# schmidtjonathan/Climate2Weather

Measured on AMD Instinct MI355X. Metric: UNet denoise steps/sec (train fwd+bwd+allreduce+AdamW+EMA windows/s), higher is better.
Workload: dtype bf16; 1 GPU; configs/sda_unet.yml default net, 5 vars x window 13 = 65 ch, 128x128, bf16 training step, 128 windows/GPU/step; global_batch=128, parallelism=dp1, params=72132929

## Files before the change

### climate2weather_amd/csrc/attention_mfma.hip

```cpp
#include <cstdlib>
#include "knobs.h"
#include "launch.h"

namespace {

constexpr int T64 = 64;
constexpr int PP = 144;

typedef __attribute__((ext_vector_type(4))) short s16x4_t;
typedef __attribute__((address_space(3))) s16x4_t lds_s16x4_t;

__device__ __forceinline__ bf16x8_t tr_frag(const char* base, int pitch, int k0, int col0, int li, int lg) {
    const int q = li >> 2, pp = li & 3;
    const char* p0 = base + (k0 + 8 * lg + q) * pitch + (col0 + pp * 4) * 2;
    const s16x4_t lo = __builtin_amdgcn_ds_read_tr16_b64_v4i16((lds_s16x4_t*)p0);
    const s16x4_t hi = __builtin_amdgcn_ds_read_tr16_b64_v4i16((lds_s16x4_t*)(p0 + 4 * pitch));
    return (bf16x8_t){lo[0], lo[1], lo[2], lo[3], hi[0], hi[1], hi[2], hi[3]};
}

template <int CTRL>
__device__ __forceinline__ float dpp_get(float v) {
    return __int_as_float(__builtin_amdgcn_update_dpp(0, __float_as_int(v), CTRL, 0xf, 0xf, false));
}
__device__ __forceinline__ float row16_sum(float v) {
    v += dpp_get<0x128>(v);
    v += dpp_get<0x124>(v);
    v += dpp_get<0x122>(v);
    return v + dpp_get<0x121>(v);
}
__device__ __forceinline__ float row16_max(float v) {
    v = fmaxf(v, dpp_get<0x128>(v));
    v = fmaxf(v, dpp_get<0x124>(v));
    v = fmaxf(v, dpp_get<0x122>(v));
    return fmaxf(v, dpp_get<0x121>(v));
}

__device__ __forceinline__ void stage_rows(char* dst, int pitch, const bf16_t* src, int ld, int C) {
    const int nch = C >> 3;
    for (int i = threadIdx.x; i < T64 * nch; i += blockDim.x) {
        const int r = i / nch, c = i - r * nch;
        *(u32x4_t*)(dst + r * pitch + c * 16) = *(const u32x4_t*)(src + (size_t)r * ld + c * 8);
    }
}

template <typename T>
__device__ __forceinline__ void strip_abt(f32x4_t (&acc)[4], const bf16_t* a, int lda, const bf16_t* b, int ldb, int ks0, int ks1, int w, int li,
                                          int lg) {
    const bf16_t* ar = a + (size_t)(16 * w + li) * lda + 8 * lg;
    const bf16_t* br = b + (size_t)li * ldb + 8 * lg;
#pragma unroll 4
    for (int ks = ks0; ks < ks1; ++ks) {
        const bf16x8_t av = *(const bf16x8_t*)(ar + 32 * ks);
#pragma unroll
        for (int n = 0; n < 4; ++n) {
            const bf16x8_t bv = *(const bf16x8_t*)(br + (size_t)(16 * n) * ldb + 32 * ks);
            acc[n] = mfma16s<T>(av, bv, acc[n]);
        }
    }
}

__device__ __forceinline__ void strip_to_lds(char* X, int w, const f32x4_t (&acc)[4], int li, int lg) {
#pragma unroll
    for (int n = 0; n < 4; ++n)
#pragma unroll
        for (int r = 0; r < 4; ++r) *(float*)(X + w * 4096 + ((4 * lg + r) * 64 + 16 * n + li) * 4) = acc[n][r];
}
__device__ __forceinline__ void strip_from_lds(const char* X, int w, f32x4_t (&acc)[4], int li, int lg) {
#pragma unroll
    for (int n = 0; n < 4; ++n)
#pragma unroll
        for (int r = 0; r < 4; ++r) acc[n][r] = *(const float*)(X + w * 4096 + ((4 * lg + r) * 64 + 16 * n + li) * 4);
}

template <typename T>
__device__ __forceinline__ void strip_times_lds(bf16_t* out, int ldo, const bf16x8_t (&a)[2], const char* M, int pitch, int ct0, int ct1, int w,
                                                int li, int lg) {
    for (int ct = ct0; ct < ct1; ++ct) {
        f32x4_t acc = {0.f, 0.f, 0.f, 0.f};
#pragma unroll
        for (int ks = 0; ks < 2; ++ks) acc = mfma16s<T>(a[ks], tr_frag(M, pitch, 32 * ks, 16 * ct, li, lg), acc);
#pragma unroll
        for (int r = 0; r < 4; ++r) out[(size_t)(16 * w + 4 * lg + r) * ldo + 16 * ct + li] = f32_to_bits16<T>(acc[r]);
    }
}

constexpr int NTA = 512;

template <typename T>
__global__ __launch_bounds__(NTA) void attn_mfma_fwd_kernel(const bf16_t* __restrict__ qkv, bf16_t* __restrict__ o, float* __restrict__ lse,
                                                            int C, float scale2) {
    extern __shared__ __attribute__((aligned(16))) char smem[];
    const int VP = C * 2 + 16;
    char* const Vl = smem;
    char* const Pl = smem + T64 * VP;
    char* const X = Pl + T64 * PP;
    const int tid = threadIdx.x, lane = tid & 63, w8 = tid >> 6, w = w8 & 3, half = w8 >> 2, li = lane & 15, lg = lane >> 4;
    const int ld = 3 * C;
    const bf16_t* base = qkv + (size_t)blockIdx.x * T64 * ld;
    stage_rows(Vl, VP, base + 2 * C, ld, C);

    f32x4_t s[4] = {};
    const int nks = C / 32, ksm = nks / 2;
    strip_abt<T>(s, base, ld, base + C, ld, half ? ksm : 0, half ? nks : ksm, w, li, lg);
    if (half) strip_to_lds(X, w, s, li, lg);
    __syncthreads();
    if (!half) {
        f32x4_t s1[4];
        strip_from_lds(X, w, s1, li, lg);
#pragma unroll
        for (int r = 0; r < 4; ++r) {
            float m = -INFINITY;
#pragma unroll
            for (int n = 0; n < 4; ++n) {
                s[n][r] = (s[n][r] + s1[n][r]) * scale2;
                m = fmaxf(m, s[n][r]);
            }
            m = row16_max(m);
            float sum = 0.f;
#pragma unroll
            for (int n = 0; n < 4; ++n) {
                s[n][r] = __expf(s[n][r] - m);
                sum += s[n][r];
            }
            sum = row16_sum(sum);
            const float inv = 1.0f / sum;
            const int row = 16 * w + 4 * lg + r;
#pragma unroll
            for (int n = 0; n < 4; ++n) *(bf16_t*)(Pl + row * PP + (16 * n + li) * 2) = f32_to_bits16<T>(s[n][r] * inv);
            if (lse != nullptr && li == 0) lse[(size_t)blockIdx.x * T64 + row] = m + __logf(sum);
        }
    }
    __syncthreads();
    bf16x8_t pa[2];
#pragma unroll
    for (int ks = 0; ks < 2; ++ks) pa[ks] = *(const bf16x8_t*)(Pl + (16 * w + li) * PP + (32 * ks + 8 * lg) * 2);
    const int nct = C / 16, ctm = nct / 2;
    strip_times_lds<T>(o + (size_t)blockIdx.x * T64 * C, C, pa, Vl, VP, half ? ctm : 0, half ? nct : ctm, w, li, lg);
}

template <typename T>
__global__ __launch_bounds__(NTA) void attn_mfma_bwd_kernel(const bf16_t* __restrict__ qkv, const bf16_t* __restrict__ d_o,
                                                            const float* __restrict__ lse, bf16_t* __restrict__ dqkv, int C, float scale2) {
    extern __shared__ __attribute__((aligned(16))) char smem[];
    const int VP = C * 2 + 16;
    char* const B0 = smem;
    char* const B1 = smem + T64 * VP;
    char* const Pl = smem + 2 * T64 * VP;
    char* const Sl = Pl + T64 * PP;
    char* const X = Pl;
    const int tid = threadIdx.x, lane = tid & 63, w8 = tid >> 6, w = w8 & 3, half = w8 >> 2, li = lane & 15, lg = lane >> 4;
    const int ld = 3 * C;
    const bf16_t* base = qkv + (size_t)blockIdx.x * T64 * ld;
    const bf16_t* dob = d_o + (size_t)blockIdx.x * T64 * C;
    bf16_t* dbase = dqkv + (size_t)blockIdx.x * T64 * ld;
    stage_rows(B0, VP, base + C, ld, C);
    stage_rows(B1, VP, dob, C, C);

    f32x4_t s[4] = {}, dp[4];
    if (!half) strip_abt<T>(s, base, ld, base + C, ld, 0, C / 32, w, li, lg);
    else strip_abt<T>(s, dob, C, base + 2 * C, ld, 0, C / 32, w, li, lg);
    if (half) strip_to_lds(X, w, s, li, lg);
    __syncthreads();
    if (!half) strip_from_lds(X, w, dp, li, lg);
    __syncthreads();
    if (!half) {
#pragma unroll
        for (int r = 0; r < 4; ++r) {
            const int row = 16 * w + 4 * lg + r;
            const float l = lse[(size_t)blockIdx.x * T64 + row];
            float delta = 0.f;
#pragma unroll
            for (int n = 0; n < 4; ++n) {
                s[n][r] = __expf(s[n][r] * scale2 - l);
                delta += s[n][r] * dp[n][r];
            }
            delta = row16_sum(delta);
#pragma unroll
            for (int n = 0; n < 4; ++n) {
                const float ds = s[n][r] * (dp[n][r] - delta) * scale2;
                *(bf16_t*)(Pl + row * PP + (16 * n + li) * 2) = f32_to_bits16<T>(s[n][r]);
                *(bf16_t*)(Sl + row * PP + (16 * n + li) * 2) = f32_to_bits16<T>(ds);
            }
        }
    }
    __syncthreads();
    const int nct = C / 16, ctm = nct / 2, ct0 = half ? ctm : 0, ct1 = half ? nct : ctm;
    bf16x8_t a[2];
#pragma unroll
    for (int ks = 0; ks < 2; ++ks) a[ks] = *(const bf16x8_t*)(Sl + (16 * w + li) * PP + (32 * ks + 8 * lg) * 2);
    strip_times_lds<T>(dbase, ld, a, B0, VP, ct0, ct1, w, li, lg);
#pragma unroll
    for (int ks = 0; ks < 2; ++ks) a[ks] = tr_frag(Pl, PP, 32 * ks, 16 * w, li, lg);
    strip_times_lds<T>(dbase + 2 * C, ld, a, B1, VP, ct0, ct1, w, li, lg);
    __syncthreads();
    stage_rows(B0, VP, base, ld, C);
    __syncthreads();
#pragma unroll
    for (int ks = 0; ks < 2; ++ks) a[ks] = tr_frag(Sl, PP, 32 * ks, 16 * w, li, lg);
    strip_times_lds<T>(dbase + C, ld, a, B0, VP, ct0, ct1, w, li, lg);
}

template <typename T>
__global__ __launch_bounds__(256, 2) void attn_mfma_fwd_blocks_kernel(const bf16_t* __restrict__ qkv, bf16_t* __restrict__ o,
                                                                       float* __restrict__ lse, int Tn, int C, float scale2) {
    extern __shared__ __attribute__((aligned(16))) char smem[];
    const int VP = C * 2 + 16;
    char* const Vl = smem;
    const int tid = threadIdx.x, lane = tid & 63, w = tid >> 6, li = lane & 15, lg = lane >> 4;
    char* const Pw = smem + T64 * VP + w * (16 * PP);
    const int ld = 3 * C, nb = Tn / T64, qb = blockIdx.x;
    const bf16_t* base = qkv + (size_t)blockIdx.y * Tn * ld;
    const bf16_t* qrow = base + (size_t)(qb * T64 + 16 * w + li) * ld + 8 * lg;

    constexpr int MAXCT = 32;
    f32x4_t oacc[MAXCT];
#pragma unroll
    for (int ct = 0; ct < MAXCT; ++ct) oacc[ct] = (f32x4_t){0.f, 0.f, 0.f, 0.f};
    float mrun[4], lrun[4];
#pragma unroll
    for (int r = 0; r < 4; ++r) { mrun[r] = -INFINITY; lrun[r] = 0.f; }

    for (int j = 0; j < nb; ++j) {
        __syncthreads();
        stage_rows(Vl, VP, base + (size_t)j * T64 * ld + 2 * C, ld, C);
        f32x4_t s[4] = {};
        {
            const bf16_t* krow = base + (size_t)(j * T64 + li) * ld + C + 8 * lg;
#pragma unroll 4
            for (int ks = 0; ks < C / 32; ++ks) {
                const bf16x8_t av = *(const bf16x8_t*)(qrow + 32 * ks);
#pragma unroll
                for (int n = 0; n < 4; ++n) {
                    const bf16x8_t bv = *(const bf16x8_t*)(krow + (size_t)(16 * n) * ld + 32 * ks);
                    s[n] = mfma16s<T>(av, bv, s[n]);
                }
            }
        }
        float alpha[4];
#pragma unroll
        for (int r = 0; r < 4; ++r) {
            float mx = -INFINITY;
#pragma unroll
            for (int n = 0; n < 4; ++n) {
                s[n][r] *= scale2;
                mx = fmaxf(mx, s[n][r]);
            }
            mx = fmaxf(row16_max(mx), mrun[r]);
            alpha[r] = __expf(mrun[r] - mx);
            float sum = 0.f;
#pragma unroll
            for (int n = 0; n < 4; ++n) {
                s[n][r] = __expf(s[n][r] - mx);
                sum += s[n][r];
            }
            lrun[r] = lrun[r] * alpha[r] + row16_sum(sum);
            mrun[r] = mx;
#pragma unroll
            for (int n = 0; n < 4; ++n) *(bf16_t*)(Pw + (4 * lg + r) * PP + (16 * n + li) * 2) = f32_to_bits16<T>(s[n][r]);
        }
        __syncthreads();
        bf16x8_t pa[2];
#pragma unroll
        for (int ks = 0; ks < 2; ++ks) pa[ks] = *(const bf16x8_t*)(Pw + li * PP + (32 * ks + 8 * lg) * 2);
#pragma unroll
        for (int ct = 0; ct < MAXCT; ++ct) {
            if (ct * 16 < C) {
#pragma unroll
                for (int r = 0; r < 4; ++r) oacc[ct][r] *= alpha[r];
#pragma unroll
                for (int ks = 0; ks < 2; ++ks)
                    oacc[ct] = mfma16s<T>(pa[ks], tr_frag(Vl, VP, 32 * ks, 16 * ct, li, lg), oacc[ct]);
            }
        }
    }
    bf16_t* ob = o + ((size_t)blockIdx.y * Tn + qb * T64 + 16 * w) * C;
#pragma unroll
    for (int r = 0; r < 4; ++r) {
        const float inv = 1.0f / lrun[r];
#pragma unroll
        for (int ct = 0; ct < MAXCT; ++ct)
            if (ct * 16 < C) ob[(size_t)(4 * lg + r) * C + 16 * ct + li] = f32_to_bits16<T>(oacc[ct][r] * inv);
        if (lse != nullptr && li == 0) lse[(size_t)blockIdx.y * Tn + qb * T64 + 16 * w + 4 * lg + r] = mrun[r] + __logf(lrun[r]);
    }
}


constexpr int MAXHCT = 16;

template <typename T>
__device__ __forceinline__ void strip_acc_lds(f32x4_t (&acc)[MAXHCT], const bf16x8_t (&a)[2], const char* M, int pitch, int ct0, int nct, int li,
                                              int lg) {
#pragma unroll
    for (int c = 0; c < MAXHCT; ++c) {
        if (c < nct) {
#pragma unroll
            for (int ks = 0; ks < 2; ++ks) acc[c] = mfma16s<T>(a[ks], tr_frag(M, pitch, 32 * ks, 16 * (ct0 + c), li, lg), acc[c]);
        }
    }
}
template <typename T>
__device__ __forceinline__ void strip_store(bf16_t* out, int ldo, const f32x4_t (&acc)[MAXHCT], int ct0, int nct, int w, int li, int lg) {
#pragma unroll
    for (int c = 0; c < MAXHCT; ++c) {
        if (c < nct) {
#pragma unroll
            for (int r = 0; r < 4; ++r) out[(size_t)(16 * w + 4 * lg + r) * ldo + 16 * (ct0 + c) + li] = f32_to_bits16<T>(acc[c][r]);
        }
    }
}

template <typename T, bool WANT_P>
__device__ __forceinline__ void block_p_ds(char* Pl, char* Sl, const f32x4_t (&s)[4], const f32x4_t (&dp)[4], const float* lse_i, const float* del_i,
                                           float scale2, int w, int li, int lg) {
#pragma unroll
    for (int r = 0; r < 4; ++r) {
        const int row = 16 * w + 4 * lg + r;
        const float l = lse_i[row], delta = del_i[row];
#pragma unroll
        for (int n = 0; n < 4; ++n) {
            const float p = __expf(s[n][r] * scale2 - l);
            if (WANT_P) *(bf16_t*)(Pl + row * PP + (16 * n + li) * 2) = f32_to_bits16<T>(p);
            *(bf16_t*)(Sl + row * PP + (16 * n + li) * 2) = f32_to_bits16<T>(p * (dp[n][r] - delta) * scale2);
        }
    }
}

template <typename T>
__global__ __launch_bounds__(NTA) void attn_mfma_bwd_kv_blocks_kernel(const bf16_t* __restrict__ qkv, const bf16_t* __restrict__ d_o,
                                                                      const float* __restrict__ lse, const float* __restrict__ delta,
                                                                      bf16_t* __restrict__ dqkv, int Tn, int C, float scale2) {
    extern __shared__ __attribute__((aligned(16))) char smem[];
    const int VP = C * 2 + 16;
    char* const B0 = smem;
    char* const B1 = smem + T64 * VP;
    char* const Pl = smem + 2 * T64 * VP;
    char* const Sl = Pl + T64 * PP;
    char* const X = Pl;
    const int tid = threadIdx.x, lane = tid & 63, w8 = tid >> 6, w = w8 & 3, half = w8 >> 2, li = lane & 15, lg = lane >> 4;
    const int ld = 3 * C, nb = Tn / T64, j = blockIdx.x;
    const bf16_t* base = qkv + (size_t)blockIdx.y * Tn * ld;
    const bf16_t* dob = d_o + (size_t)blockIdx.y * Tn * C;
    const bf16_t* kj = base + (size_t)j * T64 * ld + C;
    const bf16_t* vj = base + (size_t)j * T64 * ld + 2 * C;
    const int nct = C / 16, ctm = nct / 2, ct0 = half ? ctm : 0, nc = half ? nct - ctm : ctm;
    f32x4_t dk[MAXHCT], dv[MAXHCT];
#pragma unroll
    for (int c = 0; c < MAXHCT; ++c) dk[c] = dv[c] = (f32x4_t){0.f, 0.f, 0.f, 0.f};
    for (int i = 0; i < nb; ++i) {
        const bf16_t* qi = base + (size_t)i * T64 * ld;
        const bf16_t* doi = dob + (size_t)i * T64 * C;
        __syncthreads();
        stage_rows(B0, VP, qi, ld, C);
        stage_rows(B1, VP, doi, C, C);
        f32x4_t s[4] = {}, dp[4];
        if (!half) strip_abt<T>(s, qi, ld, kj, ld, 0, C / 32, w, li, lg);
        else strip_abt<T>(s, doi, C, vj, ld, 0, C / 32, w, li, lg);
        if (half) strip_to_lds(X, w, s, li, lg);
        __syncthreads();
        if (!half) strip_from_lds(X, w, dp, li, lg);
        __syncthreads();
        if (!half) block_p_ds<T, true>(Pl, Sl, s, dp, lse + (size_t)blockIdx.y * Tn + i * T64, delta + (size_t)blockIdx.y * Tn + i * T64, scale2, w, li, lg);
        __syncthreads();
        bf16x8_t a[2];
#pragma unroll
        for (int ks = 0; ks < 2; ++ks) a[ks] = tr_frag(Pl, PP, 32 * ks, 16 * w, li, lg);
        strip_acc_lds<T>(dv, a, B1, VP, ct0, nc, li, lg);
#pragma unroll
        for (int ks = 0; ks < 2; ++ks) a[ks] = tr_frag(Sl, PP, 32 * ks, 16 * w, li, lg);
        strip_acc_lds<T>(dk, a, B0, VP, ct0, nc, li, lg);
    }
    bf16_t* dbase = dqkv + ((size_t)blockIdx.y * Tn + (size_t)j * T64) * ld;
    strip_store<T>(dbase + C, ld, dk, ct0, nc, w, li, lg);
    strip_store<T>(dbase + 2 * C, ld, dv, ct0, nc, w, li, lg);
}

template <typename T>
__global__ __launch_bounds__(NTA) void attn_mfma_bwd_q_blocks_kernel(const bf16_t* __restrict__ qkv, const bf16_t* __restrict__ d_o,
                                                                     const float* __restrict__ lse, const float* __restrict__ delta,
                                                                     bf16_t* __restrict__ dqkv, int Tn, int C, float scale2) {
    extern __shared__ __attribute__((aligned(16))) char smem[];
    const int VP = C * 2 + 16;
    char* const B0 = smem;
    char* const Pl = smem + T64 * VP;
    char* const Sl = Pl + T64 * PP;
    char* const X = Pl;
    const int tid = threadIdx.x, lane = tid & 63, w8 = tid >> 6, w = w8 & 3, half = w8 >> 2, li = lane & 15, lg = lane >> 4;
    const int ld = 3 * C, nb = Tn / T64, i = blockIdx.x;
    const bf16_t* base = qkv + (size_t)blockIdx.y * Tn * ld;
    const bf16_t* qi = base + (size_t)i * T64 * ld;
    const bf16_t* doi = d_o + ((size_t)blockIdx.y * Tn + (size_t)i * T64) * C;
    const float* lse_i = lse + (size_t)blockIdx.y * Tn + i * T64;
    const float* del_i = delta + (size_t)blockIdx.y * Tn + i * T64;
    const int nct = C / 16, ctm = nct / 2, ct0 = half ? ctm : 0, nc = half ? nct - ctm : ctm;
    f32x4_t dq[MAXHCT];
#pragma unroll
    for (int c = 0; c < MAXHCT; ++c) dq[c] = (f32x4_t){0.f, 0.f, 0.f, 0.f};
    for (int j = 0; j < nb; ++j) {
        const bf16_t* kj = base + (size_t)j * T64 * ld + C;
        const bf16_t* vj = base + (size_t)j * T64 * ld + 2 * C;
        __syncthreads();
        stage_rows(B0, VP, kj, ld, C);
        f32x4_t s[4] = {}, dp[4];
        if (!half) strip_abt<T>(s, qi, ld, kj, ld, 0, C / 32, w, li, lg);
        else strip_abt<T>(s, doi, C, vj, ld, 0, C / 32, w, li, lg);
        if (half) strip_to_lds(X, w, s, li, lg);
        __syncthreads();
        if (!half) strip_from_lds(X, w, dp, li, lg);
        __syncthreads();
        if (!half) block_p_ds<T, false>(Pl, Sl, s, dp, lse_i, del_i, scale2, w, li, lg);
        __syncthreads();
        bf16x8_t a[2];
#pragma unroll
        for (int ks = 0; ks < 2; ++ks) a[ks] = *(const bf16x8_t*)(Sl + (16 * w + li) * PP + (32 * ks + 8 * lg) * 2);
        strip_acc_lds<T>(dq, a, B0, VP, ct0, nc, li, lg);
    }
    strip_store<T>(dqkv + ((size_t)blockIdx.y * Tn + (size_t)i * T64) * ld, ld, dq, ct0, nc, w, li, lg);
}

}

static bool is16(int dtype) { return dtype == C2W_DTYPE_BF16 || dtype == C2W_DTYPE_F16; }

bool c2w_attention_mfma_eligible(int B, int Tn, int C, int dtype) {
    return is16(dtype) && Tn == T64 && C % 32 == 0 && C <= 512 && B > 0 && !c2w_knobs().attn_valu;
}

namespace {
constexpr int AM_LDS_MAX = 160 * 1024;
template <typename T>
int fwd_launch(const void* qkv, void* o, float* lse, int B, int C, hipStream_t st) {
    const int lds = T64 * (C * 2 + 16) + T64 * PP + 4 * 4096;
    if (int rc = c2w_lds_optin<attn_mfma_fwd_kernel<T>>(AM_LDS_MAX)) return rc;
    attn_mfma_fwd_kernel<T><<<B, NTA, lds, st>>>((const bf16_t*)qkv, (bf16_t*)o, lse, C, 1.0f / sqrtf((float)C));
    return (int)hipGetLastError();
}
template <typename T>
int bwd_launch(const void* qkv, const void* d_o, const float* lse, void* dqkv, int B, int C, hipStream_t st) {
    const int lds = 2 * T64 * (C * 2 + 16) + 2 * T64 * PP;
    if (int rc = c2w_lds_optin<attn_mfma_bwd_kernel<T>>(AM_LDS_MAX)) return rc;
    attn_mfma_bwd_kernel<T><<<B, NTA, lds, st>>>((const bf16_t*)qkv, (const bf16_t*)d_o, lse, (bf16_t*)dqkv, C, 1.0f / sqrtf((float)C));
    return (int)hipGetLastError();
}
template <typename T>
int blocks_launch(const void* qkv, void* o, float* lse, int B, int Tn, int C, hipStream_t st) {
    const int lds = T64 * (C * 2 + 16) + 4 * 16 * PP;
    if (int rc = c2w_lds_optin<attn_mfma_fwd_blocks_kernel<T>>(AM_LDS_MAX)) return rc;
    attn_mfma_fwd_blocks_kernel<T><<<dim3(Tn / T64, B), 256, lds, st>>>((const bf16_t*)qkv, (bf16_t*)o, lse, Tn, C, 1.0f / sqrtf((float)C));
    return (int)hipGetLastError();
}
}

int c2w_attention_mfma_forward(const void* qkv, void* o, float* lse, int B, int C, int dtype, hipStream_t st) {
    return c2w_by_dtype16(dtype, [&](auto t) { return fwd_launch<decltype(t)>(qkv, o, lse, B, C, st); });
}

int c2w_attention_mfma_backward(const void* qkv, const void* d_o, const float* lse, void* dqkv, int B, int C, int dtype, hipStream_t st) {
    return c2w_by_dtype16(dtype, [&](auto t) { return bwd_launch<decltype(t)>(qkv, d_o, lse, dqkv, B, C, st); });
}

bool c2w_attention_mfma_blocks_eligible(int B, int Tn, int C, int dtype) {
    return is16(dtype) && Tn > T64 && Tn % T64 == 0 && Tn <= 4096 && C % 32 == 0 && C <= 512 && B > 0 && !c2w_knobs().attn_valu;
}

int c2w_attention_mfma_blocks_forward(const void* qkv, void* o, float* lse, int B, int Tn, int C, int dtype, hipStream_t st) {
    return c2w_by_dtype16(dtype, [&](auto t) { return blocks_launch<decltype(t)>(qkv, o, lse, B, Tn, C, st); });
}

namespace {
template <typename T>
int blocks_bwd_launch(const void* qkv, const void* d_o, const float* lse, const float* delta, void* dqkv, int B, int Tn, int C, hipStream_t st) {
    const int VP = C * 2 + 16;
    const int lds_kv = 2 * T64 * VP + 2 * T64 * PP, lds_q = T64 * VP + 2 * T64 * PP;
    if (int rc = c2w_lds_optin<attn_mfma_bwd_kv_blocks_kernel<T>>(AM_LDS_MAX)) return rc;
    if (int rc = c2w_lds_optin<attn_mfma_bwd_q_blocks_kernel<T>>(AM_LDS_MAX)) return rc;
    const float scale2 = 1.0f / sqrtf((float)C);
    const dim3 grid(Tn / T64, B);
    attn_mfma_bwd_kv_blocks_kernel<T><<<grid, NTA, lds_kv, st>>>((const bf16_t*)qkv, (const bf16_t*)d_o, lse, delta, (bf16_t*)dqkv, Tn, C, scale2);
    attn_mfma_bwd_q_blocks_kernel<T><<<grid, NTA, lds_q, st>>>((const bf16_t*)qkv, (const bf16_t*)d_o, lse, delta, (bf16_t*)dqkv, Tn, C, scale2);
    return (int)hipGetLastError();
}
}

int c2w_attention_mfma_blocks_backward(const void* qkv, const void* d_o, const float* lse, const float* delta, void* dqkv, int B, int Tn, int C,
                                       int dtype, hipStream_t st) {
    return c2w_by_dtype16(dtype, [&](auto t) { return blocks_bwd_launch<decltype(t)>(qkv, d_o, lse, delta, dqkv, B, Tn, C, st); });
}
```

### climate2weather_amd/csrc/conv_igemm.hip

```cpp
#include <cstdlib>

#include "conv_epilogue.h"
#include "knobs.h"
#include "launch.h"

namespace {

constexpr int BN = 128;
constexpr int WBYTES = BN * 128;
constexpr int NSLOT = 3;
template <int NW> struct GCfg {
    static constexpr int BM = 64 * NW;
    static constexpr int NTHREADS = 128 * NW;
    static constexpr int PBYTES = BM * 128;
    static constexpr int ROWS_PER_ROUND = NTHREADS / 8;
    static constexpr int WROUNDS = BN / ROWS_PER_ROUND;
    static constexpr int ROUND_BYTES = NTHREADS * 16;
};

template <typename T> struct Mma;
template <> struct Mma<bf16_t> {
    __device__ static __forceinline__ void run(const u32x4_t& a, const u32x4_t& b, f32x4_t& c) { c = mfma16<bf16_t>(a, b, c); }
};
template <> struct Mma<f16_t> {
    __device__ static __forceinline__ void run(const u32x4_t& a, const u32x4_t& b, f32x4_t& c) { c = mfma16<f16_t>(a, b, c); }
};
template <> struct Mma<float> {
    __device__ static __forceinline__ void run(const u32x4_t& a, const u32x4_t& b, f32x4_t& c) {
#pragma unroll
        for (int s = 0; s < 4; ++s)
            c = __builtin_amdgcn_mfma_f32_16x16x4f32(__uint_as_float(a[s]), __uint_as_float(b[s]), c, 0, 0, 0);
    }
};

template <typename T, int MODE, int NW>
__global__ __launch_bounds__(GCfg<NW>::NTHREADS, 2) void conv_igemm_kernel(const C2wConvArgs p) {
    constexpr int BM = GCfg<NW>::BM, NTHREADS = GCfg<NW>::NTHREADS, PBYTES = GCfg<NW>::PBYTES;
    constexpr int RPR = GCfg<NW>::ROWS_PER_ROUND, WROUNDS = GCfg<NW>::WROUNDS, RB = GCfg<NW>::ROUND_BYTES;
    constexpr int ESZ = sizeof(T);
    constexpr int NT = (MODE == C2W_CONV_1X1) ? 1 : 9;
    constexpr int CK = 128 / ESZ;
    extern __shared__ __attribute__((aligned(16))) char smem[];
    char* const Pbuf = smem;
    char* const Wbuf = smem + NSLOT * PBYTES;

    const int tid = threadIdx.x;
    const int lane = tid & 63;
    const int wid = __builtin_amdgcn_readfirstlane(tid >> 6);
    const int li = lane & 15, lg = lane >> 4;
    const int wm = wid & 1, wn = wid >> 1;

    const int nN = (p.Cout + BN - 1) / BN;
    const int nblk = gridDim.x;
    int L;
    {
        const int bid = blockIdx.x, xcd = bid & 7, q = nblk >> 3, r = nblk & 7;
        L = (xcd < r ? xcd * (q + 1) : r * (q + 1) + (xcd - r) * q) + (bid >> 3);
    }
    const int tn = L % nN, tm = L / nN;
    const int co0 = tn * BN;
    const int HWo = p.Hout * p.Wout;
    const int npix = p.B * HWo;

    bool par = false;
    int pa = 0, pw = 0, psh = 0;
    const int Wh = p.Wout >> 1, HWq = HWo >> 2, nq = npix >> 2;
    if constexpr (MODE == C2W_CONV_TS2) {
        par = ((p.Hout | p.Wout) & 1) == 0 && nq % BM == 0;
        if (par) {
            const int cls = (tm * BM) / nq;
            pa = cls < 2;
            pw = (cls & 1) == 0;
            psh = pa + pw;
        }
    }
    const int b0 = (MODE == C2W_CONV_TS2 && par) ? ((tm * BM) % nq) / HWq : (tm * BM) / HWo;
    const size_t img_bytes = (size_t)p.Hin * p.Win * p.Cin * ESZ;
    size_t xrem = (size_t)(p.B - b0) * img_bytes;
    if (xrem > 0x7fffffffu) xrem = 0x7fffffffu;
    const __amdgpu_buffer_rsrc_t rx = make_rsrc((const char*)p.x + (size_t)b0 * img_bytes, (uint32_t)xrem);
    const __amdgpu_buffer_rsrc_t rw = make_rsrc(p.w, (uint32_t)((size_t)p.wrows * NT * p.Cin * ESZ));

    auto row_pixel = [&](int Q, int& b, int& oh, int& ow) {
        if (MODE == C2W_CONV_TS2 && par) {
            const int qq = Q % nq;
            b = qq / HWq;
            const int rem = qq - b * HWq;
            const int yh = rem / Wh;
            oh = 2 * yh + pa;
            ow = 2 * (rem - yh * Wh) + pw;
        } else {
            b = Q / HWo;
            const int rem = Q - b * HWo;
            oh = rem / p.Wout;
            ow = rem - oh * p.Wout;
        }
    };

    int pb[4], pyx[4];
    uint32_t plc[4];
#pragma unroll
    for (int i = 0; i < 4; ++i) {
        const int q = (tid >> 3) + RPR * i;
        const int Q = tm * BM + q;
        int b, oh, ow;
        row_pixel(Q, b, oh, ow);
        pb[i] = (Q < npix) ? (b - b0) * p.Hin : -1;
        pyx[i] = (oh << 16) | ow;
        plc[i] = (uint32_t)(((tid & 7) ^ (q & 7)) << 4);
    }
    uint32_t wvo[WROUNDS];
#pragma unroll
    for (int i = 0; i < WROUNDS; ++i) {
        const int row = (tid >> 3) + RPR * i;
        wvo[i] = (uint32_t)(co0 + row) * (uint32_t)(NT * p.Cin * ESZ) + (uint32_t)(((tid & 7) ^ (row & 7)) << 4);
    }

    const int nchunk = p.Cin / CK;
    const int NS = (MODE == C2W_CONV_TS2 && par) ? (nchunk << psh) : nchunk * NT;

    auto issue = [&](int s, int buf) {
        int chunk, kh, kw;
        if (MODE == C2W_CONV_TS2 && par) {
            chunk = s >> psh;
            const int ti = s - (chunk << psh);
            kh = pa ? 2 * (ti >> pw) : 1;
            kw = pw ? 2 * (ti & 1) : 1;
        } else {
            chunk = s / NT;
            const int tap0 = s - chunk * NT;
            kh = tap0 / 3;
            kw = tap0 - kh * 3;
        }
        const int tap = kh * 3 + kw;
        char* const pdst = Pbuf + buf * PBYTES + wid * 1024;
#pragma unroll
        for (int i = 0; i < 4; ++i) {
            int ih, iw;
            const bool ok = src_pixel<MODE>(p, pyx[i] >> 16, pyx[i] & 0xffff, kh, kw, ih, iw) && pb[i] >= 0;
            const uint32_t voff = ok ? (uint32_t)(((pb[i] + ih) * p.Win + iw) * p.Cin) * ESZ + plc[i] : C2W_OOB;
            glds16(rx, pdst + i * RB, voff, (uint32_t)chunk * 128u);
        }
        char* const wdst = Wbuf + buf * WBYTES + wid * 1024;
        const uint32_t wso = (uint32_t)(tap * p.Cin + chunk * CK) * ESZ;
#pragma unroll
        for (int i = 0; i < WROUNDS; ++i) glds16(rw, wdst + i * RB, wvo[i], wso);
    };

    uint32_t offA[4], offB[4];
#pragma unroll
    for (int m = 0; m < 4; ++m) {
        const int row = wm * 64 + m * 16 + li;
        offA[m] = (uint32_t)(row * 128 + ((lg ^ (row & 7)) << 4));
    }
#pragma unroll
    for (int n = 0; n < 4; ++n) {
        const int row = wn * 64 + n * 16 + li;
        offB[n] = (uint32_t)(row * 128 + ((lg ^ (row & 7)) << 4));
    }

    f32x4_t acc[4][4];
#pragma unroll
    for (int m = 0; m < 4; ++m)
#pragma unroll
        for (int n = 0; n < 4; ++n) acc[m][n] = (f32x4_t){0.f, 0.f, 0.f, 0.f};

    float bv[4][4];
    epi_load_bias(p, co0 + wm * 64 + lg * 4, bv);
    issue(0, 0);
    if (NS > 1) issue(1, 1);
    int slot = 0;
    for (int s = 0; s < NS; ++s) {
        if (s + 1 < NS) {
            if constexpr (WROUNDS == 2) {
                asm volatile("s_waitcnt vmcnt(6)" ::: "memory");
            } else {
                asm volatile("s_waitcnt vmcnt(8)" ::: "memory");
            }
        } else {
            asm volatile("s_waitcnt vmcnt(0)" ::: "memory");
        }
        asm volatile("s_waitcnt lgkmcnt(0)" ::: "memory");
        __builtin_amdgcn_s_barrier();
        if (s + 2 < NS) issue(s + 2, slot >= 1 ? slot - 1 : NSLOT - 1);
        const char* const Pb = Pbuf + slot * PBYTES;
        const char* const Wb = Wbuf + slot * WBYTES;
#pragma unroll
        for (int ks = 0; ks < 2; ++ks) {
            u32x4_t a[4], b[4];
#pragma unroll
            for (int m = 0; m < 4; ++m) a[m] = *(const u32x4_t*)(Wb + (offA[m] ^ (ks * 64)));
#pragma unroll
            for (int n = 0; n < 4; ++n) b[n] = *(const u32x4_t*)(Pb + (offB[n] ^ (ks * 64)));
#pragma unroll
            for (int m = 0; m < 4; ++m)
#pragma unroll
                for (int n = 0; n < 4; ++n) Mma<T>::run(a[m], b[n], acc[m][n]);
        }
        slot = slot + 1 == NSLOT ? 0 : slot + 1;
    }

    constexpr int OS = BN * ESZ + 16;
    EpiStore<T, BM, NTHREADS> est;
    est.prefetch(p, tid, co0, [&](int row) -> long long {
        const int Q = tm * BM + row;
        if (Q >= npix) return -1;
        if (MODE == C2W_CONV_TS2 && par) {
            int b, oh, ow;
            row_pixel(Q, b, oh, ow);
            return ((long long)b * p.Hout + oh) * p.Wout + ow;
        }
        return (long long)Q;
    });
    __syncthreads();
    char* const O = smem;
    epi_acc_to_lds<T>(O, OS, acc, bv, p.act, wm * 64, wn * 64, li, lg);
    __syncthreads();
    est.finish(p, O, OS, tid);
}

template <typename T, int MODE>
__global__ void conv_naive_kernel(const C2wConvArgs p) {
    constexpr int NT = (MODE == C2W_CONV_1X1) ? 1 : 9;
    const int HWo = p.Hout * p.Wout;
    const long long total = (long long)p.B * HWo * p.Cout;
    for (long long idx = (long long)blockIdx.x * blockDim.x + threadIdx.x; idx < total; idx += (long long)gridDim.x * blockDim.x) {
        const int co = (int)(idx % p.Cout);
        const long long Q = idx / p.Cout;
        const int b = (int)(Q / HWo);
        const int rem = (int)(Q - (long long)b * HWo);
        const int oh = rem / p.Wout, ow = rem - oh * p.Wout;
        float acc = 0.f;
        for (int tap = 0; tap < NT; ++tap) {
            int ih, iw;
            if (!src_pixel<MODE>(p, oh, ow, tap / 3, tap % 3, ih, iw)) continue;
            const T* xp = (const T*)p.x + (((size_t)b * p.Hin + ih) * p.Win + iw) * p.Cin;
            const T* wp = (const T*)p.w + ((size_t)co * NT + tap) * p.Cin;
            if (co >= p.wrows) continue;
            for (int ci = 0; ci < p.Cin; ++ci) acc = fmaf(Elem<T>::ld(wp + ci), Elem<T>::ld(xp + ci), acc);
        }
        if (p.bias && co < p.wrows) acc += p.bias[co];
        if (p.act == C2W_ACT_SILU) acc = silu_f(acc);
        if (p.act == C2W_ACT_RELU) acc = relu_f(acc);
        const size_t off = (size_t)Q * p.ldy + co;
        if (p.mul) {
            float g = Elem<T>::ld((const T*)p.mul + off);
            acc *= (p.mulmode == C2W_MUL_DSILU) ? dsilu_f(g) : g;
        }
        if (p.res) acc += Elem<T>::ld((const T*)p.res + off);
        if (p.act == C2W_ACT_SILU_PAIR && p.y2) {
            Elem<T>::st((T*)p.y + off, acc);
            const float a_ = Elem<T>::ld((const T*)p.y + off);
            Elem<T>::st((T*)p.y + off, silu_f(a_));
            Elem<T>::st((T*)p.y2 + off, dsilu_f(a_));
            continue;
        }
        if (p.act == C2W_ACT_RELU_PAIR && p.y2) {
            Elem<T>::st((T*)p.y + off, acc);
            const float a_ = Elem<T>::ld((const T*)p.y + off);
            Elem<T>::st((T*)p.y + off, relu_f(a_));
            Elem<T>::st((T*)p.y2 + off, a_ > 0.f ? 1.f : 0.f);
            continue;
        }
        Elem<T>::st((T*)p.y + off, acc);
        if (p.y2) Elem<T>::st((T*)p.y2 + off, silu_f(Elem<T>::ld((const T*)p.y + off)));
    }
}

template <typename T, int MODE, int NW>
int launch_tile(const C2wConvArgs& a, long long npix, int nN, hipStream_t st) {
    typedef GCfg<NW> CF;
    constexpr int ESZ = sizeof(T);
    constexpr int lds_loop = NSLOT * (CF::PBYTES + WBYTES), lds_epi = CF::BM * (BN * ESZ + 16);
    constexpr int lds = lds_loop > lds_epi ? lds_loop : lds_epi;
    if (int rc = c2w_lds_optin<conv_igemm_kernel<T, MODE, NW>>(lds)) return rc;
    const int nM = (int)((npix + CF::BM - 1) / CF::BM);
    conv_igemm_kernel<T, MODE, NW><<<nM * nN, CF::NTHREADS, lds, st>>>(a);
    return (int)hipGetLastError();
}

template <typename T, int MODE>
int launch_mode(const C2wConvArgs& a, int naive, hipStream_t st) {
    const long long npix = (long long)a.B * a.Hout * a.Wout;
    if (naive) {
        long long total = npix * a.Cout;
        int grid = (int)((total + 255) / 256 < 65536 ? (total + 255) / 256 : 65536);
        conv_naive_kernel<T, MODE><<<grid, 256, 0, st>>>(a);
        return (int)hipGetLastError();
    }
    const int nN = (a.Cout + BN - 1) / BN;
    const bool small = ((npix + 255) / 256) * nN < c2w_cu_count();
    return small ? launch_tile<T, MODE, 2>(a, npix, nN, st) : launch_tile<T, MODE, 4>(a, npix, nN, st);
}

template <typename T>
int launch_dtype(const C2wConvArgs& a, int naive, hipStream_t st) {
    switch (a.mode) {
        case C2W_CONV_1X1: return launch_mode<T, C2W_CONV_1X1>(a, naive, st);
        case C2W_CONV_S1: return launch_mode<T, C2W_CONV_S1>(a, naive, st);
        case C2W_CONV_S2: return launch_mode<T, C2W_CONV_S2>(a, naive, st);
        case C2W_CONV_UP: return launch_mode<T, C2W_CONV_UP>(a, naive, st);
        case C2W_CONV_TS2: return launch_mode<T, C2W_CONV_TS2>(a, naive, st);
    }
    return C2W_ERR_BAD_ARG;
}

}

namespace {
C2wKnobs read_knobs() {
    C2wKnobs k;
    k.force_gather = getenv("C2W_FORCE_GATHER") != nullptr;
    k.conv_t3 = getenv("C2W_CONV_T3") ? atoi(getenv("C2W_CONV_T3")) : -1;
    k.conv_s2_patch = getenv("C2W_CONV_S2_PATCH") ? atoi(getenv("C2W_CONV_S2_PATCH")) : 0;
    k.ts2_pairs = !(getenv("C2W_TS2_PAIRS") && atoi(getenv("C2W_TS2_PAIRS")) == 0);
    k.wgrad_atomics = getenv("C2W_WGRAD_ATOMICS") != nullptr;
    k.loss_fusion = getenv("C2W_NO_LOSS_FUSION") == nullptr;
    k.half8 = getenv("C2W_NO_HALF8") == nullptr;
    k.half8_db = !(getenv("C2W_HALF8_DB") && atoi(getenv("C2W_HALF8_DB")) == 0);
    k.attn_valu = getenv("C2W_ATTN_VALU") != nullptr;
    return k;
}
C2wKnobs g_knobs = read_knobs();
}
const C2wKnobs& c2w_knobs() { return g_knobs; }
extern "C" void c2w_knobs_reload(void) { g_knobs = read_knobs(); }

extern "C" int c2w_conv_patch_supported(const C2wConvArgs* a, int dtype) {
    (void)dtype;
    return a != nullptr && c2w_conv_patch_eligible(*a) && !c2w_knobs().force_gather ? 1 : 0;
}

extern "C" int c2w_conv_pool2_supported(const C2wConvArgs* a, int dtype) {
    (void)dtype;
    if (a == nullptr || a->mode != C2W_CONV_S1 || a->res != nullptr || a->mul != nullptr || a->y2 != nullptr || a->act != C2W_ACT_NONE ||
        a->ln_x != nullptr || a->lnf_y != nullptr)
        return 0;
    return c2w_conv_patch_eligible(*a) && !c2w_conv_pair_eligible(*a) && !c2w_knobs().force_gather ? 1 : 0;
}

extern "C" int c2w_conv_lnfwd_supported(const C2wConvArgs* a, int dtype) {
    if (a == nullptr || (dtype != C2W_DTYPE_BF16 && dtype != C2W_DTYPE_F16)) return 0;
    if (a->Cout != 128 || a->ldy != 128 || a->mul != nullptr || a->y2 != nullptr || a->act != C2W_ACT_NONE || a->ln_x != nullptr) return 0;
    return c2w_conv_patch_eligible(*a) && !c2w_knobs().force_gather ? 1 : 0;
}

extern "C" int c2w_conv_lnbwd_supported(const C2wConvArgs* a, int dtype) {
    if (a == nullptr || (dtype != C2W_DTYPE_BF16 && dtype != C2W_DTYPE_F16)) return 0;
    if (a->Cout != 128 || a->ldy != 128 || a->mul != nullptr || a->y2 != nullptr || a->act != C2W_ACT_NONE) return 0;
    return c2w_conv_patch_eligible(*a) && !c2w_knobs().force_gather ? 1 : 0;
}

int c2w_conv_splitk_plan_impl(const C2wConvArgs& a, int dtype, unsigned long long* ws_bytes);
extern "C" int c2w_conv_splitk_plan(const C2wConvArgs* a, int dtype, unsigned long long* ws_bytes) {
    if (a == nullptr) return C2W_ERR_BAD_ARG;
    return c2w_conv_splitk_plan_impl(*a, dtype, ws_bytes);
}

extern "C" int c2w_conv_lnfwd_chain_supported(const C2wConvArgs* a, int dtype) {
    if (!c2w_conv_lnfwd_supported(a, dtype)) return 0;
    return a->mode == C2W_CONV_S1 && c2w_conv_patch3_wanted(*a, dtype) ? 1 : 0;
}

extern "C" int c2w_conv_loss_supported(const C2wConvArgs* a, int dtype) {
    if (a == nullptr || (dtype != C2W_DTYPE_BF16 && dtype != C2W_DTYPE_F16)) return 0;
    if (a->mode != C2W_CONV_S1 || a->wrows > 80 || a->Cout > 128 || a->ldy != 128 || a->res != nullptr || a->mul != nullptr || a->y2 != nullptr ||
        a->act != C2W_ACT_NONE || a->ln_x != nullptr || a->lnf_y != nullptr || (a->flags & C2W_CONV_POOL2) != 0)
        return 0;
    if (a->loss_sum != nullptr && (a->loss_eps == nullptr || a->loss_C <= 0 || a->loss_C != a->wrows || (a->loss_lde & 7) != 0 || a->loss_lde < a->loss_C ||
                                   a->loss_lde > 128))
        return 0;
    const C2wKnobs& k = c2w_knobs();
    return !k.force_gather && k.loss_fusion && c2w_conv_patch_eligible(*a) && c2w_conv_patch3_wanted(*a, dtype) ? 1 : 0;
}

extern "C" long long c2w_conv_det_scratch_bytes(const C2wConvArgs* a, int dtype) {
    if (a == nullptr) return C2W_ERR_BAD_ARG;
    if (a->ln_x != nullptr && a->ln_dm != nullptr) {
        if (!c2w_conv_lnbwd_supported(a, dtype)) return C2W_ERR_UNSUPPORTED;
        return (long long)a->B * (a->Hout >> 3) * (a->Wout >> 4) * 128 * (long long)sizeof(float);
    }
    if (a->loss_sum != nullptr) {
        C2wConvArgs g = *a;
        g.loss_sum = nullptr;
        if (!c2w_conv_loss_supported(&g, dtype)) return C2W_ERR_UNSUPPORTED;
        return (long long)a->B * (a->Hout >> 4) * (a->Wout >> 4) * ((a->Cout + 127) / 128) * (long long)sizeof(float);
    }
    return 0;
}

extern "C" int c2w_conv_wpacked_supported(const C2wConvArgs* a, int dtype) {
    if (a == nullptr || (dtype != C2W_DTYPE_BF16 && dtype != C2W_DTYPE_F16)) return 0;
    return !c2w_knobs().force_gather && c2w_conv_patch_eligible(*a) && c2w_conv_patch3_wanted(*a, dtype) ? 1 : 0;
}

extern "C" int c2w_conv_dispatch(const C2wConvArgs* a, int dtype) {
    if (a == nullptr) return C2W_ERR_BAD_ARG;
    const bool gather = c2w_knobs().force_gather;
    if (!gather && c2w_conv_patch_eligible(*a)) return c2w_conv_patch3_wanted(*a, dtype) ? C2W_KERNEL_PATCH_16X16 : C2W_KERNEL_PATCH_8X16;
    if (!gather && c2w_conv_pair_eligible(*a)) return C2W_KERNEL_PATCH_PAIR;
    if (!gather && c2w_conv_ts2_patch_eligible(*a)) return C2W_KERNEL_PATCH_TS2;
    if (!gather && c2w_conv_s2_patch_eligible(*a, dtype)) return C2W_KERNEL_PATCH_S2;
    return C2W_KERNEL_GATHER;
}

extern "C" int c2w_conv_forward(const C2wConvArgs* a, int dtype, int naive, void* stream) {
    if (a == nullptr || a->x == nullptr || a->w == nullptr || a->y == nullptr) return C2W_ERR_BAD_ARG;
    const int esz = dtype == C2W_DTYPE_F32 ? 4 : 2;
    const int ck = 128 / esz;
    if (a->Cin <= 0 || a->Cin % ck != 0) return C2W_ERR_BAD_SHAPE;
    if (a->Cout <= 0 || a->Cout % (16 / esz) != 0 || a->ldy % (16 / esz) != 0) return C2W_ERR_BAD_SHAPE;
    if (a->B <= 0 || a->Hin <= 0 || a->Win <= 0 || a->Hout <= 0 || a->Wout <= 0) return C2W_ERR_BAD_SHAPE;
    if (a->Hout >= 65536 || a->Wout >= 65536) return C2W_ERR_BAD_SHAPE;
    if (a->Cout > a->ldy) return C2W_ERR_BAD_SHAPE;
    if (!c2w_conv_grid_defined(*a)) return C2W_ERR_BAD_SHAPE;
    if (a->act < C2W_ACT_NONE || a->act > C2W_ACT_RELU_PAIR) return C2W_ERR_BAD_ARG;
    if ((a->act == C2W_ACT_SILU_PAIR || a->act == C2W_ACT_RELU_PAIR) && a->y2 == nullptr) return C2W_ERR_BAD_ARG;
    hipStream_t st = (hipStream_t)stream;
    if (a->ln_x != nullptr && (naive != 0 || !c2w_conv_lnbwd_supported(a, dtype))) return C2W_ERR_BAD_SHAPE;
    if (a->lnf_y != nullptr && (naive != 0 || !c2w_conv_lnfwd_supported(a, dtype))) return C2W_ERR_BAD_SHAPE;
    if ((a->ln_rstd != nullptr && a->ln_x == nullptr) || (a->lnf_rstd != nullptr && a->lnf_y == nullptr)) return C2W_ERR_BAD_ARG;
    if (a->lnf_mean != nullptr || a->res_rstd != nullptr || a->res_mean != nullptr || a->res_m != nullptr || (a->flags & C2W_CONV_NO_Y) != 0) {
        if (a->lnf_y == nullptr || (a->res_rstd == nullptr) != (a->res_mean == nullptr) || (a->res_m != nullptr && a->res_rstd == nullptr) ||
            (a->res_rstd != nullptr && a->res == nullptr))
            return C2W_ERR_BAD_ARG;
        if (naive != 0 || !c2w_conv_lnfwd_chain_supported(a, dtype)) return C2W_ERR_BAD_SHAPE;
    }
    if ((a->flags & C2W_CONV_POOL2) != 0 && (naive != 0 || !c2w_conv_pool2_supported(a, dtype))) return C2W_ERR_BAD_SHAPE;
    if (a->loss_sum != nullptr && (naive != 0 || !c2w_conv_loss_supported(a, dtype))) return C2W_ERR_BAD_SHAPE;
    if ((a->flags & C2W_CONV_DETERMINISTIC) != 0 && ((a->ln_x != nullptr && a->ln_dm != nullptr) || a->loss_sum != nullptr)) {
        const long long need = c2w_conv_det_scratch_bytes(a, dtype);
        if (need < 0 || a->det_ws == nullptr || a->det_ws_bytes < (unsigned long long)need) return C2W_ERR_BAD_ARG;
    }
    if (a->splitk > 1) {
        unsigned long long need = 0;
        if (naive != 0 || a->splitk_ws == nullptr || c2w_conv_splitk_plan_impl(*a, dtype, &need) != a->splitk || a->splitk_ws_bytes < need) return C2W_ERR_BAD_SHAPE;
    }
    if ((a->flags & C2W_CONV_WPACKED) != 0 && (naive != 0 || !c2w_conv_wpacked_supported(a, dtype))) return C2W_ERR_BAD_SHAPE;
    const bool patch = naive == 0 && !c2w_knobs().force_gather;
    if (patch && c2w_conv_patch_eligible(*a)) return c2w_conv_patch_s1(*a, dtype, st);
    if (patch && c2w_conv_pair_eligible(*a)) return c2w_conv_patch_pair(*a, dtype, st);
    if (patch && c2w_conv_ts2_patch_eligible(*a)) return c2w_conv_patch_ts2(*a, dtype, st);
    if (patch && c2w_conv_s2_patch_eligible(*a, dtype)) return c2w_conv_patch_s2(*a, dtype, st);
    if (naive == 2) naive = 0;
    return c2w_by_dtype(dtype, [&](auto t) { return launch_dtype<decltype(t)>(*a, naive, st); });
}
```

### climate2weather_amd/csrc/knobs.h

```cpp
#pragma once

struct C2wKnobs {
    bool force_gather;
    int conv_t3;
    int conv_s2_patch;
    bool ts2_pairs;
    bool wgrad_atomics;
    bool attn_valu;
    bool loss_fusion;
    bool half8;
    bool half8_db;
};

const C2wKnobs& c2w_knobs();
extern "C" void c2w_knobs_reload(void);
```

Measured before the change: 2781 windows/s.

## Split small-sequence attention fwd/bwd across two blocks per image

Adds a split mode for the single-tile (64-token) MFMA attention kernels, used when 2*B fits within the CU count. Each image now gets two workgroups instead of one. In the forward pass each block owns half the query rows and reduces QK^T partial sums across waves through LDS. In the backward pass each block recomputes the softmax and owns half the output channel tiles, staging only its slice of K/V/dO. The goal is to fill idle CUs when the batch is small, at the cost of duplicated score and softmax work in the backward pass and extra LDS reductions. The mode is on by default through a new knob.

```diff
diff --git a/climate2weather_amd/csrc/attention_mfma.hip b/climate2weather_amd/csrc/attention_mfma.hip
--- a/climate2weather_amd/csrc/attention_mfma.hip
+++ b/climate2weather_amd/csrc/attention_mfma.hip
@@ -74,11 +74,11 @@
 
 template <typename T>
 __device__ __forceinline__ void strip_times_lds(bf16_t* out, int ldo, const bf16x8_t (&a)[2], const char* M, int pitch, int ct0, int ct1, int w,
-                                                int li, int lg) {
+                                                int li, int lg, int ctl = 0) {
     for (int ct = ct0; ct < ct1; ++ct) {
         f32x4_t acc = {0.f, 0.f, 0.f, 0.f};
 #pragma unroll
-        for (int ks = 0; ks < 2; ++ks) acc = mfma16s<T>(a[ks], tr_frag(M, pitch, 32 * ks, 16 * ct, li, lg), acc);
+        for (int ks = 0; ks < 2; ++ks) acc = mfma16s<T>(a[ks], tr_frag(M, pitch, 32 * ks, 16 * (ct - ctl), li, lg), acc);
 #pragma unroll
         for (int r = 0; r < 4; ++r) out[(size_t)(16 * w + 4 * lg + r) * ldo + 16 * ct + li] = f32_to_bits16<T>(acc[r]);
     }
@@ -138,11 +138,13 @@
     strip_times_lds<T>(o + (size_t)blockIdx.x * T64 * C, C, pa, Vl, VP, half ? ctm : 0, half ? nct : ctm, w, li, lg);
 }
 
-template <typename T>
+template <typename T, bool SPLIT>
 __global__ __launch_bounds__(NTA) void attn_mfma_bwd_kernel(const bf16_t* __restrict__ qkv, const bf16_t* __restrict__ d_o,
                                                             const float* __restrict__ lse, bf16_t* __restrict__ dqkv, int C, float scale2) {
     extern __shared__ __attribute__((aligned(16))) char smem[];
-    const int VP = C * 2 + 16;
+    const int img = SPLIT ? blockIdx.x >> 1 : blockIdx.x, nct = C / 16;
+    const int cta = SPLIT && (blockIdx.x & 1) ? nct / 2 : 0, ctb = SPLIT && !(blockIdx.x & 1) ? nct / 2 : nct;
+    const int VP = (ctb - cta) * 32 + 16;
     char* const B0 = smem;
     char* const B1 = smem + T64 * VP;
     char* const Pl = smem + 2 * T64 * VP;
@@ -150,11 +152,11 @@
     char* const X = Pl;
     const int tid = threadIdx.x, lane = tid & 63, w8 = tid >> 6, w = w8 & 3, half = w8 >> 2, li = lane & 15, lg = lane >> 4;
     const int ld = 3 * C;
-    const bf16_t* base = qkv + (size_t)blockIdx.x * T64 * ld;
-    const bf16_t* dob = d_o + (size_t)blockIdx.x * T64 * C;
-    bf16_t* dbase = dqkv + (size_t)blockIdx.x * T64 * ld;
-    stage_rows(B0, VP, base + C, ld, C);
-    stage_rows(B1, VP, dob, C, C);
+    const bf16_t* base = qkv + (size_t)img * T64 * ld;
+    const bf16_t* dob = d_o + (size_t)img * T64 * C;
+    bf16_t* dbase = dqkv + (size_t)img * T64 * ld;
+    stage_rows(B0, VP, base + C + 16 * cta, ld, 16 * (ctb - cta));
+    stage_rows(B1, VP, dob + 16 * cta, C, 16 * (ctb - cta));
 
     f32x4_t s[4] = {}, dp[4];
     if (!half) strip_abt<T>(s, base, ld, base + C, ld, 0, C / 32, w, li, lg);
@@ -167,7 +169,7 @@
 #pragma unroll
         for (int r = 0; r < 4; ++r) {
             const int row = 16 * w + 4 * lg + r;
-            const float l = lse[(size_t)blockIdx.x * T64 + row];
+            const float l = lse[(size_t)img * T64 + row];
             float delta = 0.f;
 #pragma unroll
             for (int n = 0; n < 4; ++n) {
@@ -184,20 +186,20 @@
         }
     }
     __syncthreads();
-    const int nct = C / 16, ctm = nct / 2, ct0 = half ? ctm : 0, ct1 = half ? nct : ctm;
+    const int ctm = cta + (ctb - cta) / 2, ct0 = half ? ctm : cta, ct1 = half ? ctb : ctm;
     bf16x8_t a[2];
 #pragma unroll
     for (int ks = 0; ks < 2; ++ks) a[ks] = *(const bf16x8_t*)(Sl + (16 * w + li) * PP + (32 * ks + 8 * lg) * 2);
-    strip_times_lds<T>(dbase, ld, a, B0, VP, ct0, ct1, w, li, lg);
+    strip_times_lds<T>(dbase, ld, a, B0, VP, ct0, ct1, w, li, lg, cta);
 #pragma unroll
     for (int ks = 0; ks < 2; ++ks) a[ks] = tr_frag(Pl, PP, 32 * ks, 16 * w, li, lg);
-    strip_times_lds<T>(dbase + 2 * C, ld, a, B1, VP, ct0, ct1, w, li, lg);
-    __syncthreads();
-    stage_rows(B0, VP, base, ld, C);
+    strip_times_lds<T>(dbase + 2 * C, ld, a, B1, VP, ct0, ct1, w, li, lg, cta);
+    __syncthreads();
+    stage_rows(B0, VP, base + 16 * cta, ld, 16 * (ctb - cta));
     __syncthreads();
 #pragma unroll
     for (int ks = 0; ks < 2; ++ks) a[ks] = tr_frag(Sl, PP, 32 * ks, 16 * w, li, lg);
-    strip_times_lds<T>(dbase + C, ld, a, B0, VP, ct0, ct1, w, li, lg);
+    strip_times_lds<T>(dbase + C, ld, a, B0, VP, ct0, ct1, w, li, lg, cta);
 }
 
 template <typename T>
@@ -417,6 +419,69 @@
     strip_store<T>(dqkv + ((size_t)blockIdx.y * Tn + (size_t)i * T64) * ld, ld, dq, ct0, nc, w, li, lg);
 }
 
+constexpr int XPF = 68;
+
+template <typename T>
+__global__ __launch_bounds__(NTA) void attn_mfma_fwd_split_kernel(const bf16_t* __restrict__ qkv, bf16_t* __restrict__ o, float* __restrict__ lse,
+                                                                  int C, float scale2) {
+    extern __shared__ __attribute__((aligned(16))) char smem[];
+    const int VP = C * 2 + 16;
+    char* const Vl = smem;
+    char* const Pl = smem + T64 * VP;
+    float* const X = (float*)(Pl + T64 * PP);
+    const int tid = threadIdx.x, lane = tid & 63, w8 = tid >> 6, li = lane & 15, lg = lane >> 4;
+    const int img = blockIdx.x >> 1, sl = w8 & 1, w = 2 * (blockIdx.x & 1) + sl, half = (w8 >> 1) & 1, sub = w8 >> 2, j = half + 2 * sub;
+    const int ld = 3 * C;
+    const bf16_t* base = qkv + (size_t)img * T64 * ld;
+    stage_rows(Vl, VP, base + 2 * C, ld, C);
+    {
+        f32x4_t s[2] = {};
+        const int nks = C / 32, ksm = nks / 2, ks1 = half ? nks : ksm;
+        const bf16_t* ar = base + (size_t)(16 * w + li) * ld + 8 * lg;
+        const bf16_t* br = base + C + (size_t)(32 * sub + li) * ld + 8 * lg;
+#pragma unroll 4
+        for (int ks = half ? ksm : 0; ks < ks1; ++ks) {
+            const bf16x8_t av = *(const bf16x8_t*)(ar + 32 * ks);
+#pragma unroll
+            for (int n = 0; n < 2; ++n) s[n] = mfma16s<T>(av, *(const bf16x8_t*)(br + (size_t)(16 * n) * ld + 32 * ks), s[n]);
+        }
+        float* const Xw = X + (2 * sl + half) * (16 * XPF);
+#pragma unroll
+        for (int n = 0; n < 2; ++n)
+#pragma unroll
+            for (int r = 0; r < 4; ++r) Xw[(4 * lg + r) * XPF + 16 * (2 * sub + n) + li] = s[n][r];
+    }
+    __syncthreads();
+    {
+        const float* const X0 = X + (2 * sl) * (16 * XPF) + (4 * j + lg) * XPF + li;
+        const int row = 16 * w + 4 * j + lg;
+        float s[4], m = -INFINITY;
+#pragma unroll
+        for (int n = 0; n < 4; ++n) {
+            s[n] = (X0[16 * n] + X0[16 * XPF + 16 * n]) * scale2;
+            m = fmaxf(m, s[n]);
+        }
+        m = row16_max(m);
+        float sum = 0.f;
+#pragma unroll
+        for (int n = 0; n < 4; ++n) {
+            s[n] = __expf(s[n] - m);
+            sum += s[n];
+        }
+        sum = row16_sum(sum);
+        const float inv = 1.0f / sum;
+#pragma unroll
+        for (int n = 0; n < 4; ++n) *(bf16_t*)(Pl + row * PP + (16 * n + li) * 2) = f32_to_bits16<T>(s[n] * inv);
+        if (lse != nullptr && li == 0) lse[(size_t)img * T64 + row] = m + __logf(sum);
+    }
+    __syncthreads();
+    bf16x8_t pa[2];
+#pragma unroll
+    for (int ks = 0; ks < 2; ++ks) pa[ks] = *(const bf16x8_t*)(Pl + (16 * w + li) * PP + (32 * ks + 8 * lg) * 2);
+    const int nct = C / 16;
+    strip_times_lds<T>(o + (size_t)img * T64 * C, C, pa, Vl, VP, nct * j / 4, nct * (j + 1) / 4, w, li, lg);
+}
+
 }
 
 static bool is16(int dtype) { return dtype == C2W_DTYPE_BF16 || dtype == C2W_DTYPE_F16; }
@@ -427,18 +492,31 @@
 
 namespace {
 constexpr int AM_LDS_MAX = 160 * 1024;
+bool split_wanted(int B, int bit) { return (c2w_knobs().attn_split & bit) != 0 && 2 * B <= c2w_cu_count(); }
 template <typename T>
 int fwd_launch(const void* qkv, void* o, float* lse, int B, int C, hipStream_t st) {
     const int lds = T64 * (C * 2 + 16) + T64 * PP + 4 * 4096;
+    const float scale2 = 1.0f / sqrtf((float)C);
+    if (split_wanted(B, 1)) {
+        if (int rc = c2w_lds_optin<attn_mfma_fwd_split_kernel<T>>(AM_LDS_MAX)) return rc;
+        attn_mfma_fwd_split_kernel<T><<<2 * B, NTA, lds - 4 * 4096 + 4 * 16 * XPF * 4, st>>>((const bf16_t*)qkv, (bf16_t*)o, lse, C, scale2);
+        return (int)hipGetLastError();
+    }
     if (int rc = c2w_lds_optin<attn_mfma_fwd_kernel<T>>(AM_LDS_MAX)) return rc;
-    attn_mfma_fwd_kernel<T><<<B, NTA, lds, st>>>((const bf16_t*)qkv, (bf16_t*)o, lse, C, 1.0f / sqrtf((float)C));
+    attn_mfma_fwd_kernel<T><<<B, NTA, lds, st>>>((const bf16_t*)qkv, (bf16_t*)o, lse, C, scale2);
     return (int)hipGetLastError();
 }
 template <typename T>
 int bwd_launch(const void* qkv, const void* d_o, const float* lse, void* dqkv, int B, int C, hipStream_t st) {
+    const float scale2 = 1.0f / sqrtf((float)C);
+    if (split_wanted(B, 2)) {
+        if (int rc = c2w_lds_optin<attn_mfma_bwd_kernel<T, true>>(AM_LDS_MAX)) return rc;
+        attn_mfma_bwd_kernel<T, true><<<2 * B, NTA, 2 * T64 * (C + 16) + 2 * T64 * PP, st>>>((const bf16_t*)qkv, (const bf16_t*)d_o, lse, (bf16_t*)dqkv, C, scale2);
+        return (int)hipGetLastError();
+    }
     const int lds = 2 * T64 * (C * 2 + 16) + 2 * T64 * PP;
-    if (int rc = c2w_lds_optin<attn_mfma_bwd_kernel<T>>(AM_LDS_MAX)) return rc;
-    attn_mfma_bwd_kernel<T><<<B, NTA, lds, st>>>((const bf16_t*)qkv, (const bf16_t*)d_o, lse, (bf16_t*)dqkv, C, 1.0f / sqrtf((float)C));
+    if (int rc = c2w_lds_optin<attn_mfma_bwd_kernel<T, false>>(AM_LDS_MAX)) return rc;
+    attn_mfma_bwd_kernel<T, false><<<B, NTA, lds, st>>>((const bf16_t*)qkv, (const bf16_t*)d_o, lse, (bf16_t*)dqkv, C, scale2);
     return (int)hipGetLastError();
 }
 template <typename T>
diff --git a/climate2weather_amd/csrc/conv_igemm.hip b/climate2weather_amd/csrc/conv_igemm.hip
--- a/climate2weather_amd/csrc/conv_igemm.hip
+++ b/climate2weather_amd/csrc/conv_igemm.hip
@@ -319,6 +319,7 @@
     k.half8 = getenv("C2W_NO_HALF8") == nullptr;
     k.half8_db = !(getenv("C2W_HALF8_DB") && atoi(getenv("C2W_HALF8_DB")) == 0);
     k.attn_valu = getenv("C2W_ATTN_VALU") != nullptr;
+    k.attn_split = getenv("C2W_ATTN_SPLIT") ? atoi(getenv("C2W_ATTN_SPLIT")) : 3;
     return k;
 }
 C2wKnobs g_knobs = read_knobs();
diff --git a/climate2weather_amd/csrc/knobs.h b/climate2weather_amd/csrc/knobs.h
--- a/climate2weather_amd/csrc/knobs.h
+++ b/climate2weather_amd/csrc/knobs.h
@@ -7,6 +7,7 @@
     bool ts2_pairs;
     bool wgrad_atomics;
     bool attn_valu;
+    int attn_split;
     bool loss_fusion;
     bool half8;
     bool half8_db;
```

Result: no change. 2784 windows/s (median of 2 runs) (+0.1%).
